# NeLy-EPFL/DeepFly3D

Hardware: AMD Instinct MI355X
Metric: frames/sec (7-view 2D->3D) (higher is better)
Workload: dtype f32; 1 GPU; BASELINE configs[1]: 2176 frames x 7 views 256x512x3 per GPU, 2-stack hourglass fp32, arg-max + 38-joint layout + fp64 DLT; frames_per_gpu=2176, parallelism=frame-sharded x1, one packed gather, collective_executed=False

## Files before the change

deepfly3d_amd/csrc/hg_bt_wino_f32.h:

```cpp
#pragma once
#include "hg_bt_common.h"
#include "hg_bt_reg.h"
#include "hg_bt_ring_f32.h"
#include "hg_types.h"

#ifndef WN_ABL
#define WN_ABL 0
#endif

namespace hgk {

constexpr int WN_CHUNKS = 16;
constexpr int WN_PASSES = 6;
#ifndef WN_UBUF
#define WN_UBUF 3
#endif
constexpr int WN_PASS_BYTES = 4 * 4 * 1024;
constexpr int WN_U_BYTES = 64 * WN_PASS_BYTES;
constexpr int WN_U2_BYTES = (WN_CHUNKS * WN_PASSES - 64) * WN_PASS_BYTES;
constexpr int WN_W3_BYTES = BRF_W3_STAGES * BR_STAGE_BYTES;
constexpr int WN_STREAM_BYTES = WN_U_BYTES + WN_W3_BYTES;
constexpr int WN_STREAM_BYTES_L2 = WN_U_BYTES + 2 * WN_W3_BYTES;
constexpr int WN_V_BYTES = 12 * 1024;
constexpr int WN_T1_OFF = BR_RING_BYTES;
constexpr int WN_T1_BYTES = 2 * BR_T1_BYTES;
constexpr int WN_T2_BYTES = BT_TH * BT_TW * 512;
constexpr int WN_B3_OFF = WN_T1_OFF + WN_T1_BYTES;
constexpr int WN_RING2_OFF = WN_B3_OFF + 1024 + 512;
constexpr int WN_LDS_BYTES = WN_RING2_OFF + BR_RING_BYTES;
static_assert(WN_LDS_BYTES <= 160 * 1024, "one workgroup per CU");
static_assert(WN_PASSES % WN_UBUF == 0 && WN_UBUF >= 2, "a chunk's passes use the same buffers in every chunk");
static_assert(WN_V_BYTES <= BR_RING_BYTES / 2, "V buffers 0, 1 in the W3 ring's slots 0 .. 3, buffer 2 in slots 4 .. 7");
static_assert(WN_T2_BYTES <= WN_T1_BYTES, "t2 lives in the t1 region");
static_assert(WN_U2_BYTES <= BRF_NSTAGE * BR_STAGE_BYTES, "U's second part fits the direct-form stage images");

__host__ __device__ constexpr int wn_row(int pg, int q4) { return pg >= 3 ? 3 - (q4 & 1) : (q4 & 1); }
__host__ __device__ constexpr int wn_col(int pg, int q4) { return 2 * (pg % 3) + (q4 >> 1); }

__global__ __launch_bounds__(256) void bt_wino_pack_kernel(const float* __restrict__ w2, float* __restrict__ ustream, float* __restrict__ ustream2) {
    const int idx = blockIdx.x * 256 + threadIdx.x;
    if (idx >= 128 * 128) return;
    const int co = idx >> 7, ci = idx & 127;
    double g[3][3];
#pragma unroll
    for (int ky = 0; ky < 3; ++ky)
#pragma unroll
        for (int kx = 0; kx < 3; ++kx) g[ky][kx] = (double)w2[((size_t)(ky * 3 + kx) * 128 + co) * 128 + ci];
    double t[4][3];
#pragma unroll
    for (int kx = 0; kx < 3; ++kx) {
        t[0][kx] = g[0][kx];
        t[1][kx] = 0.5 * (g[0][kx] + g[1][kx] + g[2][kx]);
        t[2][kx] = 0.5 * (g[0][kx] - g[1][kx] + g[2][kx]);
        t[3][kx] = g[2][kx];
    }
    const int c = ci >> 3, s = (ci >> 2) & 1, k = ci & 3, w = co >> 5, m = (co >> 4) & 1, r = co & 15;
#pragma unroll
    for (int pg = 0; pg < 6; ++pg)
#pragma unroll
        for (int q4 = 0; q4 < 4; ++q4) {
            const double* const x = t[wn_row(pg, q4)];
            double u;
            switch (wn_col(pg, q4)) {
                case 0: u = x[0]; break;
                case 1: u = (x[0] + x[1] + x[2]) / 3.0; break;
                case 2: u = (-x[0] + x[1] - x[2]) / 3.0; break;
                case 3: u = -(16.0 * x[0] + 8.0 * x[1] + 4.0 * x[2]) / 15.0; break;
                case 4: u = (x[0] - 2.0 * x[1] + 4.0 * x[2]) / 15.0; break;
                default: u = x[2]; break;
            }
            const int P = 6 * c + 3 * s + (pg >> 1);
            const size_t off = ((size_t)((P & 63) * 4 + w) * 4 + (pg & 1) * 2 + m) * 256 + (r + 16 * k) * 4 + q4;
            (P < 64 ? ustream : ustream2)[off] = (float)u;
        }
}
__global__ __launch_bounds__(256) void bt_wino_pack_w3_kernel(const float* __restrict__ w3, unsigned char* __restrict__ stream) {
    const int idx = blockIdx.x * 256 + threadIdx.x;
    if (idx >= BRF_W3_STAGES * 512) return;
    const int k = idx >> 9, rem = idx & 511, c = rem & 3, r = rem >> 2, nh = k >> 3, k8 = k & 7;
    const int ch = 4 * (r & 31) + (r >> 5);
    *reinterpret_cast<u32x4*>(stream + (size_t)k * BR_STAGE_BYTES + br_swz(r, c)) = *reinterpret_cast<const u32x4*>(w3 + ((size_t)nh * 128 + ch) * 128 + 16 * k8 + 4 * c);
}

__device__ __forceinline__ void wn_uload4(f32x4 (&d)[4], const void* sbase, unsigned voff) {
    asm volatile("s_nop 4\n\tglobal_load_dwordx4 %0, %4, %5\n\tglobal_load_dwordx4 %1, %4, %5 offset:1024\n\t"
                 "global_load_dwordx4 %2, %4, %5 offset:2048\n\tglobal_load_dwordx4 %3, %4, %5 offset:3072"
                 : "=&v"(d[0]), "=&v"(d[1]), "=&v"(d[2]), "=&v"(d[3])
                 : "v"(voff), "s"(sbase)
                 : "memory");
}
template <int N>
__device__ __forceinline__ void wn_uwait(f32x4 (&u)[4]) {
    asm volatile("s_waitcnt vmcnt(%4)" : "+v"(u[0]), "+v"(u[1]), "+v"(u[2]), "+v"(u[3]) : "n"(N) : "memory");
}
__device__ __forceinline__ unsigned wn_far_off(unsigned off) {
    asm volatile("" : "+s"(off));
    return off;
}
__device__ __forceinline__ void wn_xload1(f32x4& d, const void* sbase, unsigned voff) {
    asm volatile("s_nop 4\n\tglobal_load_dwordx4 %0, %1, %2" : "=&v"(d) : "v"(voff), "s"(sbase) : "memory");
}
template <int STEP>
__device__ __forceinline__ void wn_xload4s(f32x4 (&d)[4], const void* sbase, unsigned voff) {
    asm volatile("s_nop 4\n\tglobal_load_dwordx4 %0, %4, %5\n\tglobal_load_dwordx4 %1, %4, %5 offset:%6\n\t"
                 "global_load_dwordx4 %2, %4, %5 offset:%7\n\tglobal_load_dwordx4 %3, %4, %5 offset:%8"
                 : "=&v"(d[0]), "=&v"(d[1]), "=&v"(d[2]), "=&v"(d[3])
                 : "v"(voff), "s"(sbase), "n"(STEP), "n"(2 * STEP), "n"(3 * STEP)
                 : "memory");
}

template <bool UP, bool ADD2 = false, bool L2 = false>
__global__ __launch_bounds__(256, 1) void bottleneck_wino_f32_kernel(BtRingArgs p) {
    static_assert(!(UP && ADD2), "the fused up-path sum is written by plain blocks");
    static_assert(!L2 || (!UP && !ADD2), "layer2 is a plain block");
    using T = float;
    constexpr int CIN = L2 ? 128 : 256, CO = 256;
    extern __shared__ __attribute__((aligned(16))) unsigned char smem[];
    unsigned char* const ring = smem;
    unsigned char* const t1_lds = smem + WN_T1_OFF;
    float* const b3_lds = reinterpret_cast<float*>(smem + WN_B3_OFF);
    float* const b2_lds = b3_lds + 256;
    const unsigned ring_addr = lds_addr(ring), t1_addr = lds_addr(t1_lds);

    const int tid = threadIdx.x, lane = tid & 63;
    const int wave = __builtin_amdgcn_readfirstlane(tid >> 6);
    const int tiles_x = p.W / BT_TW, tiles_y = p.H / BT_TH;
    const int ntiles = p.V * tiles_y * tiles_x;
    auto tile_of = [&](int vb, int& tx0, int& ty0, int& view) {
        const BtTile t = bt_tile<BT_TW, BT_TH>(vb, ntiles, tiles_x, tiles_y);
        tx0 = t.tx0, ty0 = t.ty0, view = t.view;
    };
    unsigned uoff = (unsigned)(lane * 16);
    asm volatile("" : "+v"(uoff));
    auto t1_issue = [&](int tx0, int ty0, int view) {
        bt_t1_issue_persistent<BT_HW, BT_HALO, 512, 2>(p.t1in, p.zeros, view, tx0, ty0, p.H, p.W, t1_addr, wave, uoff);
    };


    const unsigned char* const ubase = reinterpret_cast<const unsigned char*>(p.w2d) + (size_t)wave * 4096;
    const unsigned char* const ubase2 = reinterpret_cast<const unsigned char*>(p.wstream) + (size_t)wave * 4096 - (size_t)64 * WN_PASS_BYTES;
    auto uload = [&](int c, int e, f32x4 (&dst)[4]) {
        const int P = WN_PASSES * c + e;
        wn_uload4(dst, (P < 64 ? ubase : ubase2) + (size_t)P * WN_PASS_BYTES, uoff);
    };

    const int wh = wave & 1;
    unsigned rd[6], vwr, vrd;
    auto lane_consts = [&]() {
        int l = (int)(uoff >> 4);
        asm volatile("" : "+v"(l));
        const int ppc = l & 3, pte = (l >> 2) & 3, pkq = (l >> 4) & 1, ppr = 2 * (wave >> 1) + (l >> 5);
#pragma unroll
        for (int col = 0; col < 6; ++col) {
            const int hx = 4 * ppc + col, hp = (2 * ppr + wh) * BT_HW + hx;
            rd[col] = (unsigned)(hp * 256 + ((pkq ^ (hx & 15)) << 4) + 4 * pte);
        }
        vwr = (unsigned)(((pkq * 6 + 3 * wh) * 4 + pte) * 256 + (((4 * ppr + ppc) ^ (4 * pte)) << 4));
        vrd = (unsigned)((l >> 4) * 256 + (((l & 15) ^ (4 * (l >> 4))) << 4));
    };
    auto vbuf_off = [](int b) { return b == 0 ? 0 : b == 1 ? BR_RING_BYTES / 2 : WN_RING2_OFF; };
    unsigned vrd2 = 0, vwr2 = 0;
    auto vrd_of = [&](int b) { return b == 2 ? smem + vrd2 : smem + vbuf_off(b) + vrd; };
    const f32x2 cw2 = {-1.0f, wh ? 0.0f : 1.0f}, cw0 = {0.0f, wh ? -1.0f : 0.0f};
    float tR[6][3];
    unsigned ta[6];
    auto t_addr = [&](int c) {
#pragma unroll
        for (int col = 0; col < 6; ++col) {
            ta[col] = (rd[col] ^ (unsigned)((c & 7) << 5)) + (t1_addr + (unsigned)((c >> 3) * BR_T1_BYTES));
            asm volatile("" : "+v"(ta[col]));
        }
    };
    auto t_read = [&](int col) {
        typedef const __attribute__((address_space(3))) float* lds_f;
        if (WN_ABL & 512) {
            asm volatile("" : "+v"(tR[col][0]), "+v"(tR[col][1]), "+v"(tR[col][2]));
            return;
        }
#pragma unroll
        for (int t = 0; t < 3; ++t) tR[col][t] = *(lds_f)(size_t)(ta[col] + t * BT_HW * 256);
    };
    f32x4 vo[3];
    auto t_transform = [&](int c_next_addr) {
        f32x2 x[6];
#pragma unroll
        for (int col = 0; col < 6; ++col) {
            const f32x2 P = {tR[col][0], tR[col][1]};
            if (WN_ABL & 2048) {
                x[col] = P;
                continue;
            }
            x[col] = cw0 * f32x2{tR[col][0], tR[col][0]} + (cw2 * f32x2{tR[col][2], tR[col][2]} + P);
        }
        f32x2 v[6];
        if (WN_ABL & 2048) {
#pragma unroll
            for (int j = 0; j < 6; ++j) v[j] = x[j];
        } else {
            const f32x2 h = {0.5f, 0.5f}, two = {2.0f, 2.0f};
            const f32x2 d13 = x[3] - x[1], d24 = x[4] - x[2];
            v[0] = h * d13 + (((x[0] + x[4]) - two * x[2]) + d13);
            v[1] = h * x[3] + (two * x[3] + (h * x[2] + (x[4] - x[1])));
            v[2] = h * x[3] + (((x[4] + x[1]) - two * x[2]) - h * x[2]);
            v[3] = two * (x[3] - x[1]) + d24;
            v[4] = h * (x[1] - x[3]) + d24;
            v[5] = h * d24 + (((x[5] + x[1]) - two * x[3]) + d24);
        }
#pragma unroll
        for (int jp = 0; jp < 3; ++jp) vo[jp] = f32x4{v[2 * jp][0], v[2 * jp][1], v[2 * jp + 1][0], v[2 * jp + 1][1]};
        t_addr(c_next_addr);
    };
    auto v_store = [&](int buf, int jp) {
        if (WN_ABL & 1024) {
            asm volatile("" ::"v"(vo[jp]));
            return;
        }
        *reinterpret_cast<f32x4*>((buf == 2 ? smem + vwr2 : smem + vbuf_off(buf) + vwr) + jp * 1024) = vo[jp];
    };
    auto t_transform_write = [&](int buf, int c_next_addr) {
        t_transform(c_next_addr);
#pragma unroll
        for (int jp = 0; jp < 3; ++jp) v_store(buf, jp);
    };
    auto ring_slot = [](int k) { return (k & 7) < 4 ? (k & 7) * BR_STAGE_BYTES : WN_RING2_OFF + ((k & 7) - 4) * BR_STAGE_BYTES; };
    auto ring_issue8 = [&](int set) {
        unsigned wvoff = (unsigned)wave * 2048u + uoff;
        asm volatile("" : "+v"(wvoff));
#pragma unroll
        for (int k = 8 * set; k < 8 * set + 8; ++k)
            br_ring_issue(reinterpret_cast<const unsigned char*>(p.w2d) + WN_U_BYTES, k, ring_addr + (unsigned)ring_slot(k), wave, wvoff);
    };

#ifdef DF3D_BT_TIMING
    unsigned long long stamp_ = __builtin_amdgcn_s_memtime();
#endif
    int vb = blockIdx.x;
    int tx0, ty0, view;
    tile_of(vb, tx0, ty0, view);
    t1_issue(tx0, ty0, view);
    b3_lds[tid] = L2 ? p.b3[tid] + p.bd[tid] : p.b3[tid];
    if (tid < 128) b2_lds[tid] = p.b2[tid];
    bool first = true;

#pragma unroll 1
    for (;;) {
        const int vbn = vb + (int)gridDim.x;
        const bool has_next = vbn < ntiles;
        int ntx0 = 0, nty0 = 0, nview = 0;
        if (has_next) tile_of(vbn, ntx0, nty0, nview);
        const size_t ftile = (((size_t)view * p.H + ty0 + 2 * wave) * p.W + tx0) * (CO * 4);
        const size_t htile = (((size_t)view * (p.H / 2) + ty0 / 2 + wave) * (p.W / 2) + tx0 / 2) * (CO * 4);
        const unsigned char* const xtile = reinterpret_cast<const unsigned char*>(p.in) + (L2 ? ftile / 2 : ftile);

        f32x4 acc[48];
        f32x4 ufr[WN_UBUF][4];
#pragma unroll
        for (int e = 0; e < WN_UBUF - 1; ++e) uload(0, e, ufr[e]);
        if (first) asm volatile("s_waitcnt vmcnt(%0)" ::"n"(4 * (WN_UBUF - 1)) : "memory");
        first = false;
        br_barrier();
        BR_STAMP(0);
        lane_consts();
        t_addr(0);
#pragma unroll
        for (int col = 0; col < 6; ++col) t_read(col);
        t_transform_write(0, 1);
#pragma unroll
        for (int col = 0; col < 6; ++col) t_read(col);
        t_transform_write(1, 2);
        br_barrier();
        BR_STAMP(1);

        f32x4 vf[2][2];
        auto chunk = [&](int c, auto br_tag, auto first_tag) {
            constexpr int BR = decltype(br_tag)::value;
            constexpr bool FIRST = decltype(first_tag)::value;
            const int cn = c + 1 < WN_CHUNKS ? c + 1 : c;
            const int c3 = c + 3 < WN_CHUNKS ? c + 3 : WN_CHUNKS - 1;
            const unsigned char* const vb_ = vrd_of(BR);
            if (FIRST) {
#pragma unroll
                for (int g = 0; g < 2; ++g) vf[0][g] = *reinterpret_cast<const f32x4*>(vb_ + g * 1024);
            }
#pragma unroll
            for (int e = 0; e < WN_PASSES; ++e) {
                const int pp = e % 3;
                __builtin_amdgcn_sched_barrier(0);
                if (!(WN_ABL & 1)) {
                    wn_uwait<4 * (WN_UBUF - 2)>(ufr[e % WN_UBUF]);
                    const int eu = e + WN_UBUF - 1;
                    if (eu < WN_PASSES) uload(c, eu, ufr[eu % WN_UBUF]);
                    else uload(cn, eu - WN_PASSES, ufr[eu % WN_UBUF]);
                    __builtin_amdgcn_sched_barrier(0);
                }
                if (e == 3) {
                    if (BR == 0) {
                        vwr2 = vwr + wn_far_off(WN_RING2_OFF);
                        asm volatile("" : "+v"(vwr2));
                    }
                    if (BR == 1) {
                        vrd2 = vrd + wn_far_off(WN_RING2_OFF);
                        asm volatile("" : "+v"(vrd2));
                    }
                    if (!(WN_ABL & 2)) {
                        if (WN_ABL & 4096) t_transform_write((BR + 2) % 3, c3);
                        else t_transform(c3);
                    }
                    __builtin_amdgcn_sched_barrier(0);
                }
#pragma unroll
                for (int g = 0; g < 4; ++g) {
                    if (g < 2) {
                        const int en = e + 1, sn = en / 3, ppn = en % 3;
                        if (e < WN_PASSES - 1) vf[en & 1][g] = *reinterpret_cast<const f32x4*>(vb_ + (sn * 6 + 2 * ppn + g) * 1024);
                        else vf[0][g] = *reinterpret_cast<const f32x4*>(vrd_of((BR + 1) % 3) + g * 1024);
                    }
                    if (e < 2 && g < 3 && !(WN_ABL & 2)) t_read(3 * e + g);
                    if (e == 3 && g < 3 && !(WN_ABL & (2 | 4096))) v_store((BR + 2) % 3, g);
                    const int pgl = g >> 1, m = g & 1, ai = ((2 * pp + pgl) * 2 + m) * 4;
#pragma unroll
                    for (int q4 = 0; q4 < 4; ++q4) {
                        if (FIRST && e < 3)
                            acc[ai + q4] = __builtin_amdgcn_mfma_f32_16x16x4f32(ufr[e % WN_UBUF][2 * pgl + m][q4], vf[e & 1][pgl][q4], f32x4{0.0f, 0.0f, 0.0f, 0.0f}, 0, 0, 0);
                        else
                            acc[ai + q4] = __builtin_amdgcn_mfma_f32_16x16x4f32(ufr[e % WN_UBUF][2 * pgl + m][q4], vf[e & 1][pgl][q4], acc[ai + q4], 0, 0, 0);
                    }
                    __builtin_amdgcn_sched_barrier(0);
                }
            }
            if (!(WN_ABL & 4)) br_barrier();
        };
        chunk(0, std::integral_constant<int, 0>{}, std::true_type{});
#pragma unroll 1
        for (int c = 1; c < WN_CHUNKS; c += 3) {
            chunk(c, std::integral_constant<int, 1>{}, std::false_type{});
            chunk(c + 1, std::integral_constant<int, 2>{}, std::false_type{});
            chunk(c + 2, std::integral_constant<int, 0>{}, std::false_type{});
        }
        if (!(WN_ABL & 1)) {
#pragma unroll
            for (int e = 0; e < WN_UBUF - 1; ++e) wn_uwait<0>(ufr[e]);
        }

        BR_STAMP(2);
        int lane3 = (int)(uoff >> 4);
        asm volatile("" : "+v"(lane3));
        const int half3 = lane3 >> 5, l31_3 = lane3 & 31;
        const unsigned char* const wf0 = ring + br_swz(l31_3, half3);
        const unsigned char* const wf1 = ring + br_swz(l31_3, 2 + half3);
        const int py = 2 * wave + (l31_3 >> 4), px = l31_3 & 15;
        const unsigned lane_full = (unsigned)((4 * half3 * CO + 4 * l31_3) * 4);
        const unsigned lane_half = (unsigned)((2 * half3 * CO + 4 * l31_3) * 4);
        ring_issue8(0);

        if (WN_ABL & 16) {
            float keep = 0.0f;
#pragma unroll
            for (int k = 0; k < 48; ++k) keep += acc[k][0];
            *reinterpret_cast<float*>(t1_lds + lane3 * 4) = keep;
        } else {
            const int q3 = lane3 >> 4, opr = (lane3 & 15) >> 2, opc = lane3 & 3;
#pragma unroll
            for (int m = 0; m < 2; ++m) {
                f32x4 y[2][4];
                const f32x4 bb = *reinterpret_cast<const f32x4*>(b2_lds + 32 * wave + 16 * m + 4 * q3);
#pragma unroll
                for (int reg = 0; reg < 4; ++reg) {
                    float M[4][6];
#pragma unroll
                    for (int pg = 0; pg < 6; ++pg)
#pragma unroll
                        for (int q4 = 0; q4 < 4; ++q4) M[wn_row(pg, q4)][wn_col(pg, q4)] = acc[(pg * 2 + m) * 4 + q4][reg];
                    M[1][1] += bb[reg];
                    float s[2][6];
#pragma unroll
                    for (int j = 0; j < 6; ++j) {
                        s[0][j] = M[0][j] + M[1][j] + M[2][j];
                        s[1][j] = M[1][j] - M[2][j] - M[3][j];
                    }
#pragma unroll
                    for (int a = 0; a < 2; ++a) {
                        const float sa = s[a][1] + s[a][2], sb = s[a][1] - s[a][2];
                        y[a][0][reg] = br_relu(s[a][0] + sa + s[a][3] + s[a][4]);
                        y[a][1][reg] = br_relu(sb + 0.5f * s[a][3] - 2.0f * s[a][4]);
                        y[a][2][reg] = br_relu(sa + 0.25f * s[a][3] + 4.0f * s[a][4]);
                        y[a][3][reg] = br_relu(sb + 0.125f * s[a][3] - 8.0f * s[a][4] + s[a][5]);
                    }
                }
                const int ch = 8 * wave + 4 * m + q3;
#pragma unroll
                for (int a = 0; a < 2; ++a)
#pragma unroll
                    for (int b = 0; b < 4; ++b) {
                        const int yy = 2 * opr + a, xx = 4 * opc + b;
                        *reinterpret_cast<f32x4*>(t1_lds + (yy * BT_TW + xx) * 512 + (((ch ^ (xx & 15) ^ (opr & 1)) & 31) << 4)) = y[a][b];
                    }
            }
        }
        BR_STAMP(3);
        br_wait_vm(0);
        br_barrier();
        f32x16 t2[4];
        {
            const unsigned rbase = (unsigned)((py * BT_TW + px) * 512 + ((half3 ^ (px & 15) ^ (wave & 1)) << 4));
#pragma unroll
            for (int m = 0; m < 4; ++m)
#pragma unroll
                for (int g = 0; g < 4; ++g) {
                    const f32x4 v = *reinterpret_cast<const f32x4*>(t1_lds + (rbase ^ (unsigned)((8 * m + 2 * g) << 4)));
#pragma unroll
                    for (int e = 0; e < 4; ++e) t2[m][4 * g + e] = v[e];
                }
        }

        br_barrier();
        if (has_next && !(WN_ABL & 32)) t1_issue(ntx0, nty0, nview);
        f32x4 xres[1][16];
        f32x4 exv[4];
        static_assert(!(UP && ADD2), "one extra operand");
        auto res_issue = [&](int nh) {
#pragma unroll
            for (int g = 0; g < 4; ++g) {
                if (WN_ABL & 64) {
#pragma unroll
                    for (int j = 0; j < 4; ++j) xres[0][4 * g + j] = f32x4{0.0f, 0.0f, 0.0f, 0.0f};
                } else {
                    wn_uload4(*reinterpret_cast<f32x4(*)[4]>(&xres[0][4 * g]), xtile + ((size_t)(g >> 1) * p.W + 8 * (g & 1)) * (CIN * 4) + nh * 512, lane_full);
                }
            }
            if constexpr (ADD2 || UP) {
#pragma unroll
                for (int key = 0; key < 4; ++key)
                    wn_xload1(exv[key], reinterpret_cast<const unsigned char*>(ADD2 ? p.add2 : p.in2) + htile + ((key & 1) + 4 * (key >> 1)) * (CO * 4) + nh * 512, lane_half);
            }
        };
        auto res_wait = [&](auto n_tag) {
            constexpr int N = decltype(n_tag)::value;
#pragma unroll
            for (int g = 0; g < 4; ++g) wn_uwait<N>(*reinterpret_cast<f32x4(*)[4]>(&xres[0][4 * g]));
            if constexpr (ADD2 || UP) wn_uwait<N>(exv);
        };
        if constexpr (L2) {
#pragma unroll
            for (int r = 0; r < 16; ++r)
                xres[0][r] = *reinterpret_cast<const f32x4*>(xtile + (8 * r) * 4 + (unsigned)((((l31_3 >> 4) * p.W + (l31_3 & 15)) * CIN + 4 * half3) * 4));
        } else {
            res_issue(0);
        }
        BR_STAMP(4);
#pragma unroll
        for (int nh = 0; nh < 2; ++nh) {
            f32x16 o[4];
            if (nh == 1) {
                br_wait_vm(L2 ? 16 : (ADD2 || UP) ? 36 : 32);
                br_barrier();
            }
#pragma unroll
            for (int i = 0; i < 4; ++i) {
                const float bias = b3_lds[nh * 128 + 4 * l31_3 + i];
#pragma unroll
                for (int r = 0; r < 16; ++r) o[i][r] = bias;
            }
            auto kloop = [&](auto skip_tag) {
                constexpr bool SKIP = decltype(skip_tag)::value;
#pragma unroll
                for (int k8 = 0; k8 < 8; ++k8) {
                    const int tile = k8 >> 1, q2 = k8 & 1;
#pragma unroll
                    for (int jj = 0; jj < 2; ++jj)
#pragma unroll
                        for (int i = 0; i < 4; ++i) {
                            const f32x4 wf = *reinterpret_cast<const f32x4*>((jj ? wf1 : wf0) + ring_slot(k8) + i * 2048);
                            if (WN_ABL & 256) {
                                o[i][0] += wf[0];
                                continue;
                            }
                            if constexpr (SKIP) {
                                const f32x4 xa = xres[0][2 * k8 + jj];
                                mfma_quad<T>(xa[0], xa[1], xa[2], xa[3], wf, o[i]);
                            } else {
                                mfma_quad<T>(t2[tile][8 * q2 + 4 * jj], t2[tile][8 * q2 + 4 * jj + 1], t2[tile][8 * q2 + 4 * jj + 2], t2[tile][8 * q2 + 4 * jj + 3], wf, o[i]);
                            }
                        }
                }
            };
            kloop(std::false_type{});
            if constexpr (L2) {
                br_barrier();
                ring_issue8(2 + nh);
                br_wait_vm(0);
                br_barrier();
                kloop(std::true_type{});
            }
            if (nh == 0) {
                br_barrier();
                ring_issue8(1);
            }
            BR_STAMP(5 + 2 * nh);
            if constexpr (!L2) {
                if (!(WN_ABL & 64)) {
                    if (nh == 0) res_wait(std::integral_constant<int, 16>{});
                    else res_wait(std::integral_constant<int, 0>{});
                }
            }
#pragma unroll
            for (int key = 0; key < 4; ++key) {
                const int r0 = 2 * (key & 1) + 4 * (key >> 1);
                const int hoff = ((key & 1) + 4 * (key >> 1)) * (CO * 4) + nh * 512;
                f32x4 xv[4], ov[4];
#pragma unroll
                for (int t = 0; t < 4; ++t) xv[t] = L2 ? f32x4{0.0f, 0.0f, 0.0f, 0.0f} : xres[0][r0 + (t & 1) + 8 * (t >> 1)];
                if constexpr (UP) {
#pragma unroll
                    for (int t = 0; t < 4; ++t) xv[t] += exv[key];
                }
#pragma unroll
                for (int t = 0; t < 4; ++t) {
                    const int r = r0 + (t & 1) + 8 * (t >> 1);
                    ov[t] = f32x4{o[0][r], o[1][r], o[2][r], o[3][r]};
                    if constexpr (!L2) ov[t] += xv[t];
                    if constexpr (ADD2) ov[t] += exv[key];
                    const int pl0 = (r & 3) + 8 * (r >> 2);
                    if (!(WN_ABL & 128) || ov[t][0] == 12345.678f)
                        *reinterpret_cast<f32x4*>(reinterpret_cast<unsigned char*>(p.out) + ftile + ((size_t)(pl0 >> 4) * p.W + (pl0 & 15)) * (CO * 4) + nh * 512 + lane_full) = ov[t];
                }
                auto max4 = [](const f32x4 (&v)[4]) {
                    f32x4 m;
#pragma unroll
                    for (int e = 0; e < 4; ++e) m[e] = fmaxf(fmaxf(v[0][e], v[1][e]), fmaxf(v[2][e], v[3][e]));
                    return m;
                };
                if constexpr (!UP && !L2) if (p.pool_in)
                    *reinterpret_cast<f32x4*>(reinterpret_cast<unsigned char*>(p.pool_in) + htile + hoff + lane_half) = max4(xv);
                if (p.pool) *reinterpret_cast<f32x4*>(reinterpret_cast<unsigned char*>(p.pool) + htile + hoff + lane_half) = max4(ov);
            }
            BR_STAMP(6 + 2 * nh);
            if constexpr (!L2) {
                if (nh == 0) res_issue(1);
            }
        }
        if (!has_next) break;
        vb = vbn;
        tx0 = ntx0;
        ty0 = nty0;
        view = nview;
    }
}

}
```

deepfly3d_amd/csrc/hourglass.hip:

```cpp
#include "hg_plan.h"
#include "hg_launch.h"
#include "hg_weights.h"
static_assert(hgk::WN_U2_BYTES <= hgk::BRF_STREAM_BYTES, "U's second part fits the identity block's stage-image slot");
static_assert(hgk::WN_U2_BYTES <= hgk::L2F_STREAM_BYTES, "layer2: U's second part fits the stage-image slot");

namespace {

int check_forward_args(df3d_hg* h, const void* images, int n, void* ws, size_t ws_bytes) {
    DF3D_CHECK_ARG(h != nullptr, "null handle");
    if (!h->blob) {
        df3d::set_error("df3d_hg_forward: weights not set (call df3d_hg_set_weights first)");
        return DF3D_ESTATE;
    }
    DF3D_CHECK_ARG(n > 0, "n must be positive");
    DF3D_CHECK_ARG(images && ws, "null pointer");
    DF3D_CHECK_ARG(ws_bytes >= df3d_hg_workspace_bytes(h, n), "workspace too small");
    DF3D_CHECK_ARG((reinterpret_cast<uintptr_t>(ws) & 255) == 0, "workspace must be 256-byte aligned");
    return DF3D_OK;
}

}

extern "C" {

#ifdef DF3D_BT_TIMING
int df3d_dbg_ring_cycles(unsigned long long* out8) {
    if (hipMemcpyFromSymbol(out8, HIP_SYMBOL(hgk::br_dbg), 96) != hipSuccess) return -1;
    unsigned long long z[12] = {0, 0, 0, 0, 0, 0, 0, 0, 0, 0, 0, 0};
    return hipMemcpyToSymbol(HIP_SYMBOL(hgk::br_dbg), z, 96) == hipSuccess ? 0 : -1;
}
#endif

int df3d_hg_create(int dtype, int num_stacks, df3d_hg** out) {
    DF3D_CHECK_ARG(out != nullptr, "null out");
    DF3D_CHECK_ARG(dtype == DF3D_DTYPE_F32 || dtype == DF3D_DTYPE_BF16 || dtype == DF3D_DTYPE_F16 || dtype == DF3D_DTYPE_F32S, "dtype must be DF3D_DTYPE_F32, DF3D_DTYPE_BF16, DF3D_DTYPE_F16 or DF3D_DTYPE_F32S");
    DF3D_CHECK_ARG(num_stacks >= 1 && num_stacks <= 8, "num_stacks must be in [1, 8]");
    df3d_hg* h = new df3d_hg();
    h->dtype = dtype;
    h->num_stacks = num_stacks;
    h->build();
    *out = h;
    return DF3D_OK;
}

void df3d_hg_destroy(df3d_hg* h) {
    if (!h) return;
    for (auto& t : h->prof.timed) {
        (void)hipEventDestroy(t.a);
        (void)hipEventDestroy(t.b);
    }
    for (auto e : h->prof.event_pool) (void)hipEventDestroy(e);
    delete h;
}

int df3d_hg_set_input(df3d_hg* h, int height, int width) {
    DF3D_CHECK_ARG(h != nullptr, "null handle");
    DF3D_CHECK_ARG(height > 0 && width > 0 && height % 64 == 0 && width % 64 == 0, "input height and width must be multiples of 64");
    h->H = height;
    h->W = width;
    h->build();
    return DF3D_OK;
}

int df3d_hg_set_option(df3d_hg* h, const char* key, int value) {
    struct Option {
        const char* key;
        int df3d_hg::*member;
        bool (*accepts)(int value);
        const char* bad_value;
        bool replans;
        const char* after_weights;
        bool on_off = false;
    };
    constexpr auto bit = [](int v) { return v == 0 || v == 1; };
    static const Option options[] = {
        {"fuse", &df3d_hg::fuse, bit, "fuse must be 0 or 1", true, "set 'fuse' before df3d_hg_set_weights (it changes the parameter manifest)"},
        {"fuse_upadd", &df3d_hg::fuse_upadd, [](int v) { return v >= 0 && v <= 2; }, "fuse_upadd must be 0, 1 or 2", true,
         "set 'fuse_upadd' before df3d_hg_set_weights (it changes the plan)"},
        {"l1", &df3d_hg::l1, bit, "l1 must be 0 or 1", true, "set 'l1' before df3d_hg_set_weights (it changes the plan and the low-precision buffer)"},
        {"ring", &df3d_hg::ring, bit, "ring must be 0 or 1", true, "set 'ring' before df3d_hg_set_weights (it changes the low-precision buffer)"},
        {"w2d", &df3d_hg::w2d, bit, "w2d must be 0 or 1", true, "set 'w2d' before df3d_hg_set_weights (it changes the weight streams)"},
        {"ring2", &df3d_hg::ring2, bit, "ring2 must be 0 or 1", false, nullptr},
        {"split1", &df3d_hg::split1, [](int v) { return v == 0 || v == 1 || (v >= 8 && v < 16); },
         "split1 must be 0, 1 or 8 + a mask (1 identity blocks, 2 layer1, 4 layer2)", true,
         "set 'split1' before df3d_hg_set_weights (it changes the plan and the weight streams)"},
        {"wino", &df3d_hg::wino, bit, "wino must be 0 or 1", true, "set 'wino' before df3d_hg_set_weights (it changes the weight streams)"},
        {"c1res", &df3d_hg::c1res, bit, "c1res must be 0 or 1", false, nullptr},
        {"no_reuse", &df3d_hg::no_reuse, bit, "no_reuse must be 0 or 1", true, "set 'no_reuse' before df3d_hg_set_weights (it changes the workspace plan)"},
        {"chain_views", &df3d_hg::chain_views, [](int v) { return v >= 0; }, "chain_views must be >= 0", true,
         "switch 'chain_views' on or off before df3d_hg_set_weights (it changes the workspace plan)", true},
        {"row_bytes", &df3d_hg::rb_override, [](int v) { return v == 0 || v == 64 || v == 128; }, "row_bytes must be 0, 64 or 128", false, nullptr},
    };
    DF3D_CHECK_ARG(h && key, "null argument");
    for (const Option& o : options) {
        if (strcmp(key, o.key)) continue;
        DF3D_CHECK_ARG(o.accepts(value), o.bad_value);
        const bool replan = o.replans && (!o.on_off || (value > 0) != (h->*o.member > 0));
        DF3D_CHECK_ARG(!replan || h->blob == nullptr, o.after_weights);
        h->*o.member = value;
        if (replan) h->build();
        return DF3D_OK;
    }
    df3d::set_error("df3d_hg_set_option: unknown key %s", key);
    return DF3D_EINVAL;
}

int df3d_hg_num_params(const df3d_hg* h) { return h ? (int)h->params.size() : 0; }

int df3d_hg_param_desc(const df3d_hg* h, int i, df3d_hg_param* out) {
    DF3D_CHECK_ARG(h && out, "null argument");
    DF3D_CHECK_ARG(i >= 0 && i < (int)h->params.size(), "index out of range");
    *out = h->params[i];
    return DF3D_OK;
}

size_t df3d_hg_blob_floats(const df3d_hg* h) { return h ? h->blob_floats : 0; }

size_t df3d_hg_lowp_bytes(const df3d_hg* h) {
    if (!h) return 0;
    return h->stream_base() + h->stream_bytes;
}

int df3d_hg_set_weights(df3d_hg* h, const float* blob_dev, void* lowp_dev, void* stream) {
    return hg_weights::df3d_hg_set_weights(h, blob_dev, lowp_dev, df3d::as_stream(stream));
}

size_t df3d_hg_workspace_bytes(const df3d_hg* h, int n) {
    if (!h || n <= 0) return 0;
    return h->act_elems_per_view * (size_t)n * h->elem_bytes() + 256;
}

int df3d_hg_forward(df3d_hg* h, const float* images_dev, int n, float* heatmaps_dev, void* workspace_dev,
                    size_t workspace_bytes, void* stream) {
    if (int rc = check_forward_args(h, images_dev, n, workspace_dev, workspace_bytes)) return rc;
    DF3D_CHECK_ARG(heatmaps_dev != nullptr, "null heatmaps");
    unsigned char* act = reinterpret_cast<unsigned char*>(workspace_dev);
    return run_steps_dtype(h, images_dev, n, (int)h->steps.size(), heatmaps_dev, act, df3d::as_stream(stream));
}

int df3d_hg_forward_u8(df3d_hg* h, const unsigned char* frames_dev, const unsigned char* flip_dev, int n, int frame_h, int frame_w, int frame_c,
                       const float* mean3_host, const float* std3_host, int resize, float* heatmaps_dev, void* workspace_dev, size_t workspace_bytes,
                       void* stream) {
    if (int rc = check_forward_args(h, frames_dev, n, workspace_dev, workspace_bytes)) return rc;
    DF3D_CHECK_ARG(heatmaps_dev != nullptr && mean3_host && std3_host, "null pointer");
    DF3D_CHECK_ARG(frame_h > 0 && frame_w > 0 && (frame_c == 1 || frame_c == 3), "bad frame shape (C must be 1 or 3)");
    DF3D_CHECK_ARG(resize >= DF3D_RESIZE_BILINEAR && resize <= DF3D_RESIZE_AREA, "resize must be one of DF3D_RESIZE_*");
    hgk::StemU8 u;
    u.nm.resize = resize;
    u.frames = frames_dev;
    u.flip = flip_dev;
    u.FH = frame_h;
    u.FW = frame_w;
    u.FC = frame_c;
    for (int c = 0; c < 3; ++c) {
        DF3D_CHECK_ARG(std3_host[c] != 0.0f, "std must be non-zero");
        u.nm.mean[c] = mean3_host[c];
        u.nm.inv_std[c] = 1.0f / std3_host[c];
    }
    h->u8in = u;
    unsigned char* act = reinterpret_cast<unsigned char*>(workspace_dev);
    const int rc = run_steps_dtype(h, nullptr, n, (int)h->steps.size(), heatmaps_dev, act, df3d::as_stream(stream));
    h->u8in.frames = nullptr;
    return rc;
}

int df3d_hg_work(const df3d_hg* h, int n, double* flops, double* bytes) {
    DF3D_CHECK_ARG(h && flops && bytes, "null argument");
    *flops = h->flops_per_view * n;
    *bytes = h->elems_per_view * n * h->elem_bytes();
    return DF3D_OK;
}

int df3d_hg_profile(df3d_hg* h, int enable) {
    DF3D_CHECK_ARG(h != nullptr, "null handle");
    h->prof.profiling = enable != 0;
    for (auto& t : h->prof.timed) {
        h->prof.event_pool.push_back(t.a);
        h->prof.event_pool.push_back(t.b);
    }
    h->prof.timed.clear();
    return DF3D_OK;
}

int df3d_hg_profile_count(const df3d_hg* h) { return h ? (int)h->prof.kernel_names.size() : 0; }

int df3d_hg_profile_read(df3d_hg* h, int kernel_class, char* name_buf, int buflen, double* ms, double* flops, double* bytes, double* bytes_m1,
                         int* launches) {
    DF3D_CHECK_ARG(h && name_buf && buflen > 0 && ms && flops && bytes && bytes_m1 && launches, "null argument");
    DF3D_CHECK_ARG(kernel_class >= 0 && kernel_class < (int)h->prof.kernel_names.size(), "kernel_class out of range");
    snprintf(name_buf, buflen, "%s", h->prof.kernel_names[kernel_class].c_str());
    *ms = *flops = *bytes = *bytes_m1 = 0.0;
    *launches = 0;
    for (auto& t : h->prof.timed) {
        if (t.cls != kernel_class) continue;
        DF3D_HIP(hipEventSynchronize(t.b));
        float e = 0.f;
        DF3D_HIP(hipEventElapsedTime(&e, t.a, t.b));
        *ms += e;
        *flops += t.w.flops;
        *bytes += t.w.bytes;
        *bytes_m1 += t.w.bytes_m1;
        *launches += 1;
    }
    return DF3D_OK;
}

int df3d_hg_profile_executed_flops(df3d_hg* h, int kernel_class, double* flops_executed) {
    DF3D_CHECK_ARG(h && flops_executed, "null argument");
    DF3D_CHECK_ARG(kernel_class >= 0 && kernel_class < (int)h->prof.kernel_names.size(), "kernel_class out of range");
    *flops_executed = 0.0;
    for (auto& t : h->prof.timed)
        if (t.cls == kernel_class) *flops_executed += t.w.flops_executed;
    return DF3D_OK;
}

int df3d_hg_num_steps(const df3d_hg* h) { return h ? (int)h->steps.size() : 0; }

double df3d_hg_step_m1_bytes(const df3d_hg* h, int step, int n) {
    if (!h || step < 0 || step >= (int)h->steps.size() || n <= 0) return 0.0;
    return h->steps[step].m1_elems * n * h->elem_bytes();
}

int df3d_hg_step_desc(const df3d_hg* h, int step, char* name_buf, int buflen, int* hwc) {
    DF3D_CHECK_ARG(h && name_buf && hwc && buflen > 0, "null argument");
    DF3D_CHECK_ARG(step >= 0 && step < (int)h->steps.size(), "step out of range");
    const Step& st = h->steps[step];
    snprintf(name_buf, buflen, "%s", st.name.c_str());
    if (st.out >= 0) {
        const TensorDesc& t = h->tensors[st.out];
        hwc[0] = t.h;
        hwc[1] = t.w;
        hwc[2] = t.c;
    } else {
        hwc[0] = h->H / 4;
        hwc[1] = h->W / 4;
        hwc[2] = h->classes;
    }
    return DF3D_OK;
}

int df3d_hg_forward_upto(df3d_hg* h, const float* images_dev, int n, int upto, float* out_dev, void* workspace_dev,
                         size_t workspace_bytes, void* stream) {
    if (int rc = check_forward_args(h, images_dev, n, workspace_dev, workspace_bytes)) return rc;
    DF3D_CHECK_ARG(upto >= 1 && upto <= (int)h->steps.size(), "upto out of range");
    DF3D_CHECK_ARG(out_dev != nullptr, "null output");
    const Step& st = h->steps[upto - 1];
    unsigned char* act = reinterpret_cast<unsigned char*>(workspace_dev);
    hipStream_t s = df3d::as_stream(stream);
    if (int rc = run_steps_dtype(h, images_dev, n, upto, out_dev, act, s)) return rc;
    if (st.out < 0) return DF3D_OK;
    const TensorDesc& t = h->tensors[st.out];
    const long long pixels = (long long)n * t.h * t.w;
    const long long total = pixels * t.c;
    const void* src = act + t.off * (size_t)n * h->elem_bytes();
    with_elem_type(h->dtype, [&](auto e) {
        hipLaunchKernelGGL((export_kernel<StorageT<decltype(e)>>), dim3((unsigned)((total + 255) / 256)), dim3(256), 0, s, src, out_dev, pixels,
                           t.c, t.pitch);
    });
    DF3D_LAUNCH_CHECK();
    return DF3D_OK;
}

}
```

Measured before the change: 748.2 frames/s.

## Interleave residual and next-tile halo loads into the Winograd bottleneck k-loop

Replaces the bulk t1_issue of the next tile's halo and the block-wise residual loads with small slices issued between k8 steps of the output GEMM loop. Residual loads for each half are spread over the first two k8 steps, and halo pieces over the rest. Vmcnt waits are adjusted to match. The goal is to hide global-load latency behind the k-loop math and smooth out VMEM queue pressure; the risk is waitcnt miscounting or the extra scheduling barriers slowing the compute loop. It also adds per-phase timing stamps that compile only under the debug macro.

```diff
diff --git a/deepfly3d_amd/csrc/hg_bt_wino_f32.h b/deepfly3d_amd/csrc/hg_bt_wino_f32.h
--- a/deepfly3d_amd/csrc/hg_bt_wino_f32.h
+++ b/deepfly3d_amd/csrc/hg_bt_wino_f32.h
@@ -9,6 +9,22 @@
 #endif
 
 namespace hgk {
+
+enum WnStamp {
+    WNS_ENTRY, WNS_FIRST_V, WNS_PHASE2, WNS_OUT_TRANSFORM, WNS_WAIT_RING_A, WNS_BARRIER_T2, WNS_T2_READS, WNS_K_A, WNS_RING_REQ_B, WNS_WAIT_RES_A, WNS_EPILOGUE_A,
+    WNS_WAIT_RING_B, WNS_K_B, WNS_WAIT_RES_B, WNS_EPILOGUE_B, WNS_COUNT
+};
+#ifdef DF3D_BT_TIMING
+__device__ unsigned long long wn_dbg[WNS_COUNT];
+#define WN_STAMP(k)                                                    \
+    do {                                                               \
+        const unsigned long long now_ = __builtin_amdgcn_s_memtime(); \
+        wn_t_[k] += now_ - stamp_;                                     \
+        stamp_ = now_;                                                 \
+    } while (0)
+#else
+#define WN_STAMP(k) do { } while (0)
+#endif
 
 constexpr int WN_CHUNKS = 16;
 constexpr int WN_PASSES = 6;
@@ -109,6 +125,40 @@
                  : "memory");
 }
 
+struct WnHaloWalk {
+    int hx, hy;
+};
+__device__ __forceinline__ void wn_halo_begin(WnHaloWalk& h, int wave, unsigned uoff) {
+    int lane_ = (int)(uoff >> 4);
+    asm volatile("" : "+v"(lane_));
+    const int hp0 = 4 * wave + (lane_ >> 4);
+    h.hy = hp0 / BT_HW;
+    h.hx = hp0 - h.hy * BT_HW;
+}
+__device__ __forceinline__ void wn_halo_piece(WnHaloWalk& h, int k, const void* t1in, const void* zeros, int view, int tx0, int ty0, int H, int W, unsigned t1_addr,
+                                              int wave, unsigned uoff) {
+    static_assert(BT_HW >= 16, "one wrap per step of 16 halo pixels");
+    const int pc = wave + 4 * k;
+    if (4 * k + 3 < BT_HALO / 4 || pc < BT_HALO / 4) {
+        int lane_ = (int)(uoff >> 4);
+        asm volatile("" : "+v"(lane_));
+        const unsigned char* const tin = reinterpret_cast<const unsigned char*>(t1in) + (size_t)view * H * W * 512;
+        const unsigned char* const zer = reinterpret_cast<const unsigned char*>(zeros);
+        const int y = ty0 - 1 + h.hy, x = tx0 - 1 + h.hx;
+        const bool ok = (unsigned)y < (unsigned)H && (unsigned)x < (unsigned)W;
+        const unsigned c16 = (unsigned)(((lane_ & 15) ^ (h.hx & 15)) << 4);
+        const unsigned in_view = (unsigned)((y * W + x) * 512) + c16;
+        const unsigned char* const src = (ok ? tin : zer) + (ok ? in_view : c16);
+        br_glds_piece64(src, t1_addr + (unsigned)(pc * 1024));
+        br_glds_piece64(src + (ok ? 256u : 0u), t1_addr + (unsigned)(BT_HALO * 256 + pc * 1024));
+    }
+    h.hx += 16;
+    if (h.hx >= BT_HW) {
+        h.hx -= BT_HW;
+        ++h.hy;
+    }
+}
+
 template <bool UP, bool ADD2 = false, bool L2 = false>
 __global__ __launch_bounds__(256, 1) void bottleneck_wino_f32_kernel(BtRingArgs p) {
     static_assert(!(UP && ADD2), "the fused up-path sum is written by plain blocks");
@@ -232,6 +282,7 @@
     };
 
 #ifdef DF3D_BT_TIMING
+    unsigned long long wn_t_[WNS_COUNT] = {};
     unsigned long long stamp_ = __builtin_amdgcn_s_memtime();
 #endif
     int vb = blockIdx.x;
@@ -259,7 +310,7 @@
         if (first) asm volatile("s_waitcnt vmcnt(%0)" ::"n"(4 * (WN_UBUF - 1)) : "memory");
         first = false;
         br_barrier();
-        BR_STAMP(0);
+        WN_STAMP(WNS_ENTRY);
         lane_consts();
         t_addr(0);
 #pragma unroll
@@ -269,7 +320,7 @@
         for (int col = 0; col < 6; ++col) t_read(col);
         t_transform_write(1, 2);
         br_barrier();
-        BR_STAMP(1);
+        WN_STAMP(WNS_FIRST_V);
 
         f32x4 vf[2][2];
         auto chunk = [&](int c, auto br_tag, auto first_tag) {
@@ -342,7 +393,7 @@
             for (int e = 0; e < WN_UBUF - 1; ++e) wn_uwait<0>(ufr[e]);
         }
 
-        BR_STAMP(2);
+        WN_STAMP(WNS_PHASE2);
         int lane3 = (int)(uoff >> 4);
         asm volatile("" : "+v"(lane3));
         const int half3 = lane3 >> 5, l31_3 = lane3 & 31;
@@ -397,9 +448,11 @@
                     }
             }
         }
-        BR_STAMP(3);
+        WN_STAMP(WNS_OUT_TRANSFORM);
         br_wait_vm(0);
+        WN_STAMP(WNS_WAIT_RING_A);
         br_barrier();
+        WN_STAMP(WNS_BARRIER_T2);
         f32x16 t2[4];
         {
             const unsigned rbase = (unsigned)((py * BT_TW + px) * 512 + ((half3 ^ (px & 15) ^ (wave & 1)) << 4));
@@ -414,13 +467,14 @@
         }
 
         br_barrier();
-        if (has_next && !(WN_ABL & 32)) t1_issue(ntx0, nty0, nview);
+        WN_STAMP(WNS_T2_READS);
+        const bool halo_next = has_next && !(WN_ABL & 32);
         f32x4 xres[1][16];
         f32x4 exv[4];
         static_assert(!(UP && ADD2), "one extra operand");
-        auto res_issue = [&](int nh) {
-#pragma unroll
-            for (int g = 0; g < 4; ++g) {
+        auto res_issue_part = [&](int nh, int g0, int ng) {
+#pragma unroll
+            for (int g = g0; g < g0 + ng; ++g) {
                 if (WN_ABL & 64) {
 #pragma unroll
                     for (int j = 0; j < 4; ++j) xres[0][4 * g + j] = f32x4{0.0f, 0.0f, 0.0f, 0.0f};
@@ -430,9 +484,20 @@
             }
             if constexpr (ADD2 || UP) {
 #pragma unroll
-                for (int key = 0; key < 4; ++key)
+                for (int key = g0; key < g0 + ng; ++key)
                     wn_xload1(exv[key], reinterpret_cast<const unsigned char*>(ADD2 ? p.add2 : p.in2) + htile + ((key & 1) + 4 * (key >> 1)) * (CO * 4) + nh * 512, lane_half);
             }
+        };
+        WnHaloWalk halo_walk = {0, 0};
+        if (halo_next) wn_halo_begin(halo_walk, wave, uoff);
+        auto vm_slice = [&](int nh, int k8) {
+            __builtin_amdgcn_sched_barrier(0);
+            if (k8 < 2) {
+                if constexpr (!L2) res_issue_part(nh, 2 * k8, 2);
+            } else if (halo_next) {
+                wn_halo_piece(halo_walk, 6 * nh + k8 - 2, p.t1in, p.zeros, nview, ntx0, nty0, p.H, p.W, t1_addr, wave, uoff);
+            }
+            __builtin_amdgcn_sched_barrier(0);
         };
         auto res_wait = [&](auto n_tag) {
             constexpr int N = decltype(n_tag)::value;
@@ -444,15 +509,13 @@
 #pragma unroll
             for (int r = 0; r < 16; ++r)
                 xres[0][r] = *reinterpret_cast<const f32x4*>(xtile + (8 * r) * 4 + (unsigned)((((l31_3 >> 4) * p.W + (l31_3 & 15)) * CIN + 4 * half3) * 4));
-        } else {
-            res_issue(0);
-        }
-        BR_STAMP(4);
+        }
 #pragma unroll
         for (int nh = 0; nh < 2; ++nh) {
             f32x16 o[4];
             if (nh == 1) {
-                br_wait_vm(L2 ? 16 : (ADD2 || UP) ? 36 : 32);
+                br_wait_vm(16);
+                WN_STAMP(WNS_WAIT_RING_B);
                 br_barrier();
             }
 #pragma unroll
@@ -466,11 +529,14 @@
 #pragma unroll
                 for (int k8 = 0; k8 < 8; ++k8) {
                     const int tile = k8 >> 1, q2 = k8 & 1;
+                    if constexpr (!SKIP) vm_slice(nh, k8);
 #pragma unroll
                     for (int jj = 0; jj < 2; ++jj)
 #pragma unroll
                         for (int i = 0; i < 4; ++i) {
-                            const f32x4 wf = *reinterpret_cast<const f32x4*>((jj ? wf1 : wf0) + ring_slot(k8) + i * 2048);
+                            f32x4 wf;
+                            if (WN_ABL & 8192) asm volatile("" : "=v"(wf));
+                            else wf = *reinterpret_cast<const f32x4*>((jj ? wf1 : wf0) + ring_slot(k8) + i * 2048);
                             if (WN_ABL & 256) {
                                 o[i][0] += wf[0];
                                 continue;
@@ -492,16 +558,19 @@
                 br_barrier();
                 kloop(std::true_type{});
             }
+            WN_STAMP(nh == 0 ? WNS_K_A : WNS_K_B);
             if (nh == 0) {
                 br_barrier();
                 ring_issue8(1);
-            }
-            BR_STAMP(5 + 2 * nh);
+                WN_STAMP(WNS_RING_REQ_B);
+            }
             if constexpr (!L2) {
                 if (!(WN_ABL & 64)) {
-                    if (nh == 0) res_wait(std::integral_constant<int, 16>{});
-                    else res_wait(std::integral_constant<int, 0>{});
-                }
+                    if (nh == 1) res_wait(std::integral_constant<int, 0>{});
+                    else if (halo_next) res_wait(std::integral_constant<int, 16 + 12>{});
+                    else res_wait(std::integral_constant<int, 16>{});
+                }
+                WN_STAMP(nh == 0 ? WNS_WAIT_RES_A : WNS_WAIT_RES_B);
             }
 #pragma unroll
             for (int key = 0; key < 4; ++key) {
@@ -534,10 +603,7 @@
                     *reinterpret_cast<f32x4*>(reinterpret_cast<unsigned char*>(p.pool_in) + htile + hoff + lane_half) = max4(xv);
                 if (p.pool) *reinterpret_cast<f32x4*>(reinterpret_cast<unsigned char*>(p.pool) + htile + hoff + lane_half) = max4(ov);
             }
-            BR_STAMP(6 + 2 * nh);
-            if constexpr (!L2) {
-                if (nh == 0) res_issue(1);
-            }
+            WN_STAMP(nh == 0 ? WNS_EPILOGUE_A : WNS_EPILOGUE_B);
         }
         if (!has_next) break;
         vb = vbn;
@@ -545,6 +611,12 @@
         ty0 = nty0;
         view = nview;
     }
-}
-
-}
+#ifdef DF3D_BT_TIMING
+    if (tid == 0) {
+#pragma unroll
+        for (int k = 0; k < WNS_COUNT; ++k) atomicAdd(&wn_dbg[k], wn_t_[k]);
+    }
+#endif
+}
+
+}
diff --git a/deepfly3d_amd/csrc/hourglass.hip b/deepfly3d_amd/csrc/hourglass.hip
--- a/deepfly3d_amd/csrc/hourglass.hip
+++ b/deepfly3d_amd/csrc/hourglass.hip
@@ -28,6 +28,12 @@
     if (hipMemcpyFromSymbol(out8, HIP_SYMBOL(hgk::br_dbg), 96) != hipSuccess) return -1;
     unsigned long long z[12] = {0, 0, 0, 0, 0, 0, 0, 0, 0, 0, 0, 0};
     return hipMemcpyToSymbol(HIP_SYMBOL(hgk::br_dbg), z, 96) == hipSuccess ? 0 : -1;
+}
+int df3d_dbg_wino_cycles(unsigned long long* out, int count) {
+    if (count != hgk::WNS_COUNT) return -1;
+    if (hipMemcpyFromSymbol(out, HIP_SYMBOL(hgk::wn_dbg), sizeof(unsigned long long) * hgk::WNS_COUNT) != hipSuccess) return -1;
+    const unsigned long long z[hgk::WNS_COUNT] = {};
+    return hipMemcpyToSymbol(HIP_SYMBOL(hgk::wn_dbg), z, sizeof(z)) == hipSuccess ? 0 : -1;
 }
 #endif
 
```

New measurement: 754.7 frames/s, median of 6. No clear change (+0.9%).
